# TGAC/KAT

Measured on AMD Instinct MI355X. Metric: k-mers/sec (whole node) for kat comp reads-vs-assembly k=27, higher is better.
Workload: dtype u64

## Files before the change

kat_amd/csrc/kg_partition.hpp:

```cpp
#pragma once
#include "kg_kernels.hpp"
#include "kg_l1_lean.hpp"

#include <cstddef>
#include <type_traits>

namespace kg {

constexpr int PART_BLOCK = 1024;
constexpr int PART_ITEMS = BASES_PER_LANE;
constexpr int TILE_ITEMS = PART_BLOCK * PART_ITEMS;
constexpr int L1_TILE_BYTES = TILE_ITEMS;
constexpr int L1_TILE_STARTS = L1_TILE_BYTES - CHUNK_OVERLAP;
constexpr int L1_LANES_WITH_STARTS = L1_TILE_STARTS / PART_ITEMS;

__device__ __forceinline__ void lds_barrier() { asm volatile("s_waitcnt lgkmcnt(0)\n\ts_barrier" ::: "memory"); }
__device__ __forceinline__ void spill_put(uint64_t* __restrict__ spill, unsigned long long* __restrict__ spill_n, uint64_t cap, uint64_t key) {
    const unsigned long long at = atomicAdd(spill_n, 1ULL);
    if (at < cap) spill[at] = key;
}

struct PartGeom {
    uint32_t R, S;
    uint32_t P1, P2;
// ... 1140 lines not shown
    static_assert(U == 4, "a lane takes one group of the level-2 buffer: four items");
    const uint32_t S = g.S;
    unsigned long long* rk = reinterpret_cast<unsigned long long*>(lds_raw);
    uint32_t* rc = reinterpret_cast<uint32_t*>(lds_raw + (size_t)S * 8);
    const uint32_t tid = threadIdx.x, lane = tid & 63, wave = tid >> 6;
    unsigned long long* wqk = reinterpret_cast<unsigned long long*>(lds_raw + (size_t)S * 12) + (size_t)wave * QCAP;
    uint32_t* wqs = reinterpret_cast<uint32_t*>(lds_raw + (size_t)S * 12 + (size_t)NW * QCAP * 8) + (size_t)wave * QCAP;
    uint32_t new_distinct = 0;
    u32x4 kq[KP], cq[CP];
    __shared__ unsigned long long s_next_chunk;

    const uint32_t r_hi = g.b_hi * g.P2;
    auto run_end = [&](uint32_t r) -> uint64_t {
        if (bend && (r + 1) % g.P2 == 0) return bend[r / g.P2];
        return off2[r + 1];
    };
    auto next_region = [&](uint32_t from) {
        uint32_t r = from;
        while (r < r_hi && (cnt2 ? cnt2[r] == 0 : off2[r] == run_end(r))) r += gridDim.x;
        return r;
    };
    auto prefetch = [&](uint32_t r) {
        const uint64_t base = (uint64_t)r * S;
#pragma unroll
        for (int u = 0; u < KP; ++u) { const uint32_t i = (u * BLOCK + tid) * 2; kq[u] = *reinterpret_cast<const u32x4*>(t.keys + base + (i < S ? i : 0)); }
#pragma unroll
        for (int u = 0; u < CP; ++u) { const uint32_t i = (u * BLOCK + tid) * 4; cq[u] = *reinterpret_cast<const u32x4*>(t.counts + base + (i < S ? i : 0)); }
    };

    uint32_t r = next_region(g.b_lo * g.P2 + blockIdx.x);
    if (r < r_hi) prefetch(r);
    while (r < r_hi) {
        const uint64_t beg = off2[r], end = cnt2 ? beg + cnt2[r] : run_end(r);
        const uint64_t base = (uint64_t)r * S;
        const unsigned long long t_top = now();
#pragma unroll
        for (int u = 0; u < KP; ++u) { const uint32_t i = (u * BLOCK + tid) * 2; if (i < S) *reinterpret_cast<u32x4*>(rk + i) = kq[u]; }
#pragma unroll
        for (int u = 0; u < CP; ++u) { const uint32_t i = (u * BLOCK + tid) * 4; if (i < S) *reinterpret_cast<u32x4*>(rc + i) = cq[u]; }
        const uint32_t rn = next_region(r + gridDim.x);
        const uint32_t rd1 = r >> g.l2, rd2 = r & (g.P2 - 1);

        for (uint64_t sbeg = beg; sbeg < end; sbeg += seg_len) {
            const uint64_t n_run = (end - sbeg < seg_len ? end - sbeg : seg_len);
            if (tid == 0) s_next_chunk = NW;
            lds_barrier();
#pragma unroll 1
            for (int u = 0; u < CP; ++u) {
                const uint32_t i = (u * BLOCK + tid) * 4;
                if (i >= S) break;
                const u32x4 c = *reinterpret_cast<const u32x4*>(rc + i);
                if (!((c.x | c.y | c.z | c.w) & 0x80000000u)) continue;
#pragma unroll 1
                for (uint32_t j = 0; j < 4; ++j)
                    if (rc[i + j] & 0x80000000u) { rc[i + j] -= 0x80000000u; ovf_add(t, rk[i + j], 0x80000000ULL); }
            }
            lds_barrier();
            st[0] += now() - t_top;

            uint32_t q_n = 0;
            auto add1 = [&](uint32_t slot) { (void)__hip_atomic_fetch_add(&rc[slot], 1u, __ATOMIC_RELAXED, __HIP_MEMORY_SCOPE_WORKGROUP); };
            auto drain_pass = [&](bool fin ) {
                const uint32_t take = q_n < 64 ? q_n : 64;
                q_n -= take;
                bool live = lane < take;
                unsigned long long key = EMPTY; uint32_t slot = 0, budget = 0;
                if (live) { key = wqk[q_n + lane]; const uint32_t s = wqs[q_n + lane]; slot = s & 0xFFFF; budget = s >> 16; }
#pragma unroll 1
                for (int rr = 0; rr < AP2_LANE_PROBES; ++rr) {
                    const int busy = __popcll(__ballot(live));
                    if (busy == 0 || (busy < 8 && (fin || rr >= 4))) break;
                    if (live) {
                        unsigned long long c0 = rk[slot];
                        if (c0 == EMPTY) {
                            c0 = atomicCAS(&rk[slot], (unsigned long long)EMPTY, key);
                            if (c0 == EMPTY) { ++new_distinct; c0 = key; }
                        }
                        if (c0 == key) { add1(slot); live = false; }
                        else {
                            slot = slot + 1 == S ? 0 : slot + 1;
                            if (--budget == 0) { spill_put(spill, spill_n, g.spill_cap, key); live = false; }
                        }
                    }
                }
                const bool lng = live && (fin || S - budget >= (uint32_t)(AP2_LANE_PROBES + NR));
                {
                    const bool back = live && !lng;
                    const unsigned long long m = __ballot(back);
                    if (m) {
                        const uint32_t at = q_n + __builtin_amdgcn_mbcnt_hi((uint32_t)(m >> 32), __builtin_amdgcn_mbcnt_lo((uint32_t)m, 0));
                        if (back) { wqk[at] = key; wqs[at] = slot | (budget << 16); }
                        q_n += (uint32_t)__popcll(m);
                    }
                }
                unsigned long long todo = __ballot(lng);
#pragma unroll 1
                while (todo) {
                    const int src = __ffsll((long long)todo) - 1;
                    todo &= todo - 1;
                    const unsigned long long ck = lane_value((uint64_t)key, src);
                    uint32_t cs = lane_value(slot, src);
                    int cb = (int)lane_value(budget, src);
#pragma unroll 1
                    for (;;) {
                        uint32_t idx = cs + lane; if (idx >= S) idx -= S;
                        const unsigned long long c0 = rk[idx];
                        const unsigned long long mk = __ballot(c0 == ck), me = __ballot(c0 == EMPTY);
                        if (!(mk | me)) {
                            cb -= 64; cs = cs + 64 >= S ? cs + 64 - S : cs + 64;
                            if (cb <= 0) { if (lane == 0) spill_put(spill, spill_n, g.spill_cap, ck); break; }
                            continue;
                        }
                        const int first = __ffsll((long long)(mk | me)) - 1;
                        if (first >= cb) { if (lane == 0) spill_put(spill, spill_n, g.spill_cap, ck); break; }
                        unsigned long long got = ck;
                        if (!((mk >> first) & 1)) {
                            unsigned long long old = EMPTY;
                            if ((int)lane == first) old = atomicCAS(&rk[idx], (unsigned long long)EMPTY, ck);
                            old = lane_value((uint64_t)old, first);
                            if (old == EMPTY) { if ((int)lane == first) ++new_distinct; }
                            else got = old;
                        }
                        if (got == ck) { if ((int)lane == first) add1(idx); break; }
                        cb -= first; cs = cs + first >= S ? cs + first - S : cs + first;
                    }
                }
            };

            const uint64_t n_chunks = (n_run + CH - 1) / CH;
            const uint64_t n_grp = (n_run + 3) >> 2, g0 = sbeg >> 2;
            unsigned long long cur[U];
            u32x4 c_lo, n_lo;
            typename HiGroup<HB>::type c_hi{}, n_hi{};
            bool c_in, n_in;
            const L2Run<HB> run(l2_buf, g0);
            { const uint64_t gi = (uint64_t)wave * 64 + lane; c_in = gi < n_grp; run.load(c_in ? (uint32_t)gi : 0u, c_lo, c_hi); }
            auto grab = [&]() -> uint64_t {
                unsigned long long v = 0;
                if (lane == 0) v = atomicAdd(&s_next_chunk, 1ULL);
                return lane_value((uint64_t)v, 0);
            };
            for (uint64_t c = wave; c < n_chunks;) {
                const unsigned long long t_a = now();
                const uint64_t c_next = DYN ? grab() : c + NW;
                {
                    const uint64_t gi = c_next * 64 + lane;
                    n_in = gi < n_grp;
                    run.load(n_in ? (uint32_t)gi : 0u, n_lo, n_hi);
                }
                uint32_t slot[U];
                bool pend[U];
#pragma unroll
                for (int u = 0; u < U; ++u) {
                    const uint64_t rem = ((uint64_t)hi_of_group<HB>(c_hi, u) << 32) | (u == 0 ? c_lo.x : u == 1 ? c_lo.y : u == 2 ? c_lo.z : c_lo.w);
                    pend[u] = c_in && rem != L2Fmt<HB>::NONE;
                    slot[u] = place_offset(rem, g.pl, S);
                    cur[u] = place_key_d(rd1, rd2, rem, g.pl);
                    if (TEST_SPILL && spill_mod && pend[u] && __umulhi((uint32_t)(mix64(cur[u]) >> 32), spill_mod) == 0) { spill_put(spill, spill_n, g.spill_cap, cur[u]); pend[u] = false; }
                }
                const unsigned long long t_b = now();
#pragma unroll
                for (int rr = 0; rr < NR; ++rr) {
                    unsigned long long seen[U];
#pragma unroll
                    for (int u = 0; u < U; ++u) { seen[u] = EMPTY; if (pend[u]) seen[u] = rk[slot[u]]; }
                    bool claim[U];
#pragma unroll
                    for (int u = 0; u < U; ++u) {
                        const bool hit = pend[u] && seen[u] == cur[u];
                        if (hit) add1(slot[u]);
                        pend[u] = pend[u] && !hit;
                        claim[u] = pend[u] && seen[u] == EMPTY;
                        const uint32_t nx = slot[u] + 1 == S ? 0 : slot[u] + 1;
                        slot[u] = (pend[u] && !claim[u]) ? nx : slot[u];
                    }
                    bool any_claim = false;
#pragma unroll
                    for (int u = 0; u < U; ++u) any_claim = any_claim || claim[u];
                    if (INLINE_CLAIM && __any(any_claim)) {
                        unsigned long long got[U];
#pragma unroll
                        for (int u = 0; u < U; ++u) { got[u] = 0; if (claim[u]) got[u] = atomicCAS(&rk[slot[u]], (unsigned long long)EMPTY, cur[u]); }
#pragma unroll
                        for (int u = 0; u < U; ++u) {
                            if (claim[u]) {
                                if (got[u] == EMPTY) ++new_distinct;
                                const bool mine = got[u] == EMPTY || got[u] == cur[u];
                                if (mine) add1(slot[u]);
                                pend[u] = !mine;
                                if (!mine) slot[u] = slot[u] + 1 == S ? 0 : slot[u] + 1;
                            }
                        }
                    }
                }
                if (STAMP) { __builtin_amdgcn_s_waitcnt(0); }
                const unsigned long long t_c = now();
                unsigned long long pm_u[U];
                uint32_t total = 0;
#pragma unroll
                for (int u = 0; u < U; ++u) { pm_u[u] = __ballot(pend[u]); total += (uint32_t)__popcll(pm_u[u]); }
                if (total <= QCAP - 64) {
                    uint32_t at = q_n;
#pragma unroll
                    for (int u = 0; u < U; ++u) {
                        if (pend[u]) {
                            const uint32_t i = at + __builtin_amdgcn_mbcnt_hi((uint32_t)(pm_u[u] >> 32), __builtin_amdgcn_mbcnt_lo((uint32_t)pm_u[u], 0));
                            wqk[i] = cur[u]; wqs[i] = slot[u] | ((S - NR) << 16);
                        }
                        at += (uint32_t)__popcll(pm_u[u]);
                    }
                    q_n += total;
                } else {
                    uint32_t pm = 0;
#pragma unroll
                    for (int u = 0; u < U; ++u) pm |= pend[u] ? 1u << u : 0u;
#pragma unroll 1
                    for (int it = 0; it < U; ++it) {
                        const bool p = pm & 1;
                        const unsigned long long m = __ballot(p);
                        if (m) {
                            while (q_n > QCAP - 64) drain_pass(false);
                            const uint32_t at = q_n + __builtin_amdgcn_mbcnt_hi((uint32_t)(m >> 32), __builtin_amdgcn_mbcnt_lo((uint32_t)m, 0));
                            if (p) { wqk[at] = cur[0]; wqs[at] = slot[0] | ((S - NR) << 16); }
                            q_n += (uint32_t)__popcll(m);
                        }
                        pm >>= 1;
#pragma unroll
                        for (int u = 0; u + 1 < U; ++u) { cur[u] = cur[u + 1]; slot[u] = slot[u + 1]; }
                    }
                }
                const bool last = c_next >= n_chunks;
                while (q_n > (last ? 0u : 64u)) drain_pass(last);
                c_lo = n_lo; c_hi = n_hi; c_in = n_in;
                c = c_next;
                if (STAMP) { const unsigned long long t_d = now(); st[1] += t_b - t_a; st[2] += t_c - t_b; st[3] += t_d - t_c; }
            }
            if (sbeg + seg_len < end) lds_barrier();
        }
        if (rn < r_hi) prefetch(rn);
        const unsigned long long t_w = now();

        lds_barrier();
        const unsigned long long t_x = now();
#pragma unroll
        for (int u = 0; u < KP; ++u) { const uint32_t i = (u * BLOCK + tid) * 2; if (i < S) *reinterpret_cast<u32x4*>(t.keys + base + i) = *reinterpret_cast<const u32x4*>(rk + i); }
#pragma unroll
        for (int u = 0; u < CP; ++u) { const uint32_t i = (u * BLOCK + tid) * 4; if (i < S) *reinterpret_cast<u32x4*>(t.counts + base + i) = *reinterpret_cast<const u32x4*>(rc + i); }
        lds_barrier();
        if (STAMP) { st[4] += t_x - t_w; st[5] += now() - t_x; st[6] += 1; }
        r = rn;
    }
    if (STAMP && tid == 0 && stamps) for (int i = 0; i < 7; ++i) atomicAdd(&stamps[i], st[i]);
    flush_distinct(t, new_distinct);
}

constexpr int APK_LANE_PROBES = 12;
constexpr uint32_t APK_SLOT_SHIFT = 44;

template <int BLOCK, int KP , int HB, bool INLINE_CLAIM = false, bool TEST_SPILL = false,
          bool PF = true ,
          int NR = 3 ,
          bool STAMP = false ,
          int UG = 1 >
__global__ void __launch_bounds__(BLOCK, 4)
k_p3_apply_pk(DevTable t, PartGeom g, const uint64_t* __restrict__ off2, const uint8_t* __restrict__ l2_buf,
              uint64_t* __restrict__ spill, unsigned long long* __restrict__ spill_n, const uint32_t* __restrict__ cnt2, const uint64_t* __restrict__ bend,
              uint32_t qcap , uint64_t seg_len ,
              uint32_t spill_mod,
              uint32_t zero_fill ) {
    extern __shared__ __attribute__((aligned(16))) unsigned char lds_raw[];
    constexpr int NW = BLOCK / 64, U = 4 * UG;
    constexpr uint32_t CH = 64 * U;
    const uint32_t S = g.S, cb = g.cbits;
    const uint64_t cmask = pk_cmask(cb), half = pk_half(cb), rem_mask = (1ULL << APK_SLOT_SHIFT) - 1;
    unsigned long long* rk = reinterpret_cast<unsigned long long*>(lds_raw);
    const uint32_t tid = threadIdx.x, lane = tid & 63, wave = tid >> 6;
    unsigned long long* wq = rk + S + (size_t)wave * qcap;
    uint32_t new_distinct = 0;
    u32x4 kq[KP];
    __shared__ unsigned long long s_next_chunk;

    const uint32_t r_hi = g.b_hi * g.P2;
    auto run_end = [&](uint32_t r) -> uint64_t {
        if (bend && (r + 1) % g.P2 == 0) return bend[r / g.P2];
        return off2[r + 1];
    };
    auto next_region = [&](uint32_t from) {
        uint32_t r = from;
        while (r < r_hi && !zero_fill && (cnt2 ? cnt2[r] == 0 : off2[r] == run_end(r))) r += gridDim.x;
        return r;
    };
    auto prefetch = [&](uint32_t r) {
        if (zero_fill) return;
        const uint64_t base = (uint64_t)r * S;
#pragma unroll
        for (int u = 0; u < KP; ++u) { const uint32_t i = (u * BLOCK + tid) * 2; kq[u] = *reinterpret_cast<const u32x4*>(t.keys + base + (i < S ? i : 0)); }
    };
    auto next_slot = [&](uint32_t s) -> uint32_t { return s + 1 == S ? 0 : s + 1; };
    uint32_t* rk32 = reinterpret_cast<uint32_t*>(rk);
    auto add1 = [&](uint32_t slot) { (void)__hip_atomic_fetch_add(&rk32[2 * slot], 1u, __ATOMIC_RELAXED, __HIP_MEMORY_SCOPE_WORKGROUP); };

    unsigned long long st[7] = {0, 0, 0, 0, 0, 0, 0};
    auto now = [&]() -> unsigned long long { return STAMP ? (unsigned long long)clock64() : 0ULL; };
    uint32_t r = next_region(g.b_lo * g.P2 + blockIdx.x);
    if (PF && r < r_hi) prefetch(r);
    while (r < r_hi) {
        const uint64_t beg = off2[r], end = cnt2 ? beg + cnt2[r] : run_end(r);
        const uint64_t base = (uint64_t)r * S;
        const unsigned long long t_fill = now();
        if (!PF) prefetch(r);
        if (zero_fill) {
#pragma unroll
            for (int u = 0; u < KP; ++u) { const uint32_t i = (u * BLOCK + tid) * 2; if (i < S) *reinterpret_cast<u32x4*>(rk + i) = u32x4{0u, 0u, 0u, 0u}; }
        } else {
#pragma unroll
            for (int u = 0; u < KP; ++u) { const uint32_t i = (u * BLOCK + tid) * 2; if (i < S) *reinterpret_cast<u32x4*>(rk + i) = kq[u]; }
        }
        const uint32_t rn = next_region(r + gridDim.x);
        const uint32_t rd1 = r >> g.l2, rd2 = r & (g.P2 - 1);
        auto spill_rem = [&](uint64_t rem) { spill_put(spill, spill_n, g.spill_cap, place_key_d(rd1, rd2, rem, g.pl)); };

        for (uint64_t sbeg = beg; sbeg < end; sbeg += seg_len) {
            const uint64_t n_run = (end - sbeg < seg_len ? end - sbeg : seg_len);
            if (tid == 0) s_next_chunk = NW;
            lds_barrier();
            const unsigned long long t_walk = now();
            st[0] += t_walk - t_fill;

            uint32_t q_n = 0;
            auto drain_pass = [&](bool fin ) {
                const unsigned long long t_dr = now();
                struct DrainStamp { unsigned long long& acc; unsigned long long t0; bool on; __device__ ~DrainStamp() { if (on) acc += (unsigned long long)clock64() - t0; } } drain_stamp{st[2], t_dr, STAMP};
                const uint32_t take = q_n < 64 ? q_n : 64;
                q_n -= take;
                bool live = lane < take;
                uint64_t rem = 0; uint32_t slot = 0, budget = 0;
                if (live) {
                    const unsigned long long e = wq[q_n + lane];
                    rem = e & rem_mask; slot = (uint32_t)(e >> APK_SLOT_SHIFT);
                    const uint32_t home = place_offset(rem, g.pl, S);
                    budget = S - (slot >= home ? slot - home : slot + S - home);
                }
#pragma unroll 1
                for (int rr = 0; rr < APK_LANE_PROBES; ++rr) {
                    const int busy = __popcll(__ballot(live));
                    if (busy == 0 || (busy < 8 && (fin || rr >= 4))) break;
                    if (live) {
                        unsigned long long w = rk[slot];
                        if (w == 0) {
                            w = atomicCAS(&rk[slot], 0ULL, (unsigned long long)((rem << cb) | 1ULL));
                            if (w == 0) { ++new_distinct; live = false; }
                        }
                        if (live) {
                            if ((w >> cb) == rem) { add1(slot); live = false; }
                            else {
                                slot = next_slot(slot);
                                if (--budget == 0) { spill_rem(rem); live = false; }
                            }
                        }
                    }
                }
                const bool lng = live && (fin || S - budget >= (uint32_t)(APK_LANE_PROBES + NR));
                {
                    const bool back = live && !lng;
                    const unsigned long long m = __ballot(back);
                    if (m) {
                        const uint32_t at = q_n + __builtin_amdgcn_mbcnt_hi((uint32_t)(m >> 32), __builtin_amdgcn_mbcnt_lo((uint32_t)m, 0));
                        if (back) wq[at] = rem | ((unsigned long long)slot << APK_SLOT_SHIFT);
                        q_n += (uint32_t)__popcll(m);
                    }
                }
                unsigned long long todo = __ballot(lng);
#pragma unroll 1
                while (todo) {
                    const int src = __ffsll((long long)todo) - 1;
                    todo &= todo - 1;
                    const unsigned long long ck = lane_value((uint64_t)rem, src);
                    uint32_t cs = lane_value(slot, src);
                    int cbud = (int)lane_value(budget, src);
#pragma unroll 1
                    for (;;) {
                        uint32_t idx = cs + lane; if (idx >= S) idx -= S;
                        const unsigned long long w = rk[idx];
                        const unsigned long long mk = __ballot(w != 0 && (w >> cb) == ck), me = __ballot(w == 0);
                        if (!(mk | me)) {
                            cbud -= 64; cs = cs + 64 >= S ? cs + 64 - S : cs + 64;
                            if (cbud <= 0) { if (lane == 0) spill_rem(ck); break; }
                            continue;
                        }
                        const int first = __ffsll((long long)(mk | me)) - 1;
                        if (first >= cbud) { if (lane == 0) spill_rem(ck); break; }
                        if ((mk >> first) & 1) { if ((int)lane == first) add1(idx); break; }
                        unsigned long long old = 0;
                        if ((int)lane == first) old = atomicCAS(&rk[idx], 0ULL, (unsigned long long)((ck << cb) | 1ULL));
                        old = lane_value((uint64_t)old, first);
                        if (old == 0) { if ((int)lane == first) ++new_distinct; break; }
                        if ((old >> cb) == ck) { if ((int)lane == first) add1(idx); break; }
                        cbud -= first; cs = cs + first >= S ? cs + first - S : cs + first;
                    }
                }
            };

            const uint64_t n_chunks = (n_run + CH - 1) / CH;
            const uint64_t n_grp = (n_run + 3) >> 2, g0 = sbeg >> 2;
            u32x4 c_lo[UG], n_lo[UG];
            typename HiGroup<HB>::type c_hi[UG], n_hi[UG];
            bool c_in[UG], n_in[UG];
            const L2Run<HB> run(l2_buf, g0);
#pragma unroll
            for (int gq = 0; gq < UG; ++gq) {
                const uint64_t gi = ((uint64_t)wave * UG + gq) * 64 + lane;
                c_in[gq] = gi < n_grp; c_hi[gq] = typename HiGroup<HB>::type{}; n_hi[gq] = typename HiGroup<HB>::type{};
                run.load(c_in[gq] ? (uint32_t)gi : 0u, c_lo[gq], c_hi[gq]);
            }
            auto grab = [&]() -> uint64_t {
                unsigned long long v = 0;
                if (lane == 0) v = atomicAdd(&s_next_chunk, 1ULL);
                return lane_value((uint64_t)v, 0);
            };
            for (uint64_t c = wave; c < n_chunks;) {
                const uint64_t c_next = grab();
#pragma unroll
                for (int gq = 0; gq < UG; ++gq) {
                    const uint64_t gi = (c_next * UG + gq) * 64 + lane;
                    n_in[gq] = gi < n_grp;
                    run.load(n_in[gq] ? (uint32_t)gi : 0u, n_lo[gq], n_hi[gq]);
                }
                uint64_t rem[U];
                uint32_t slot[U];
                bool pend[U];
#pragma unroll
                for (int u = 0; u < U; ++u) {
                    const int gq = u >> 2, q = u & 3;
                    rem[u] = ((uint64_t)hi_of_group<HB>(c_hi[gq], q) << 32) | (q == 0 ? c_lo[gq].x : q == 1 ? c_lo[gq].y : q == 2 ? c_lo[gq].z : c_lo[gq].w);
                    pend[u] = c_in[gq] && rem[u] != L2Fmt<HB>::NONE;
                    slot[u] = place_offset(rem[u], g.pl, S);
                    if (TEST_SPILL && spill_mod && pend[u] && __umulhi((uint32_t)(mix64(place_key_d(rd1, rd2, rem[u], g.pl)) >> 32), spill_mod) == 0) { spill_rem(rem[u]); pend[u] = false; }
                }
#pragma unroll
                for (int rr = 0; rr < NR; ++rr) {
                    unsigned long long seen[U];
#pragma unroll
                    for (int u = 0; u < U; ++u) seen[u] = rk[slot[u]];
                    bool claim[U];
#pragma unroll
                    for (int u = 0; u < U; ++u) {
                        const bool hit = pend[u] && seen[u] != 0 && (seen[u] >> cb) == rem[u];
                        (void)__hip_atomic_fetch_add(&rk32[2 * slot[u]], hit ? 1u : 0u, __ATOMIC_RELAXED, __HIP_MEMORY_SCOPE_WORKGROUP);
                        pend[u] = pend[u] && !hit;
                        claim[u] = pend[u] && seen[u] == 0;
                        slot[u] = (pend[u] && !claim[u]) ? next_slot(slot[u]) : slot[u];
                    }
                    bool any_claim = false;
#pragma unroll
                    for (int u = 0; u < U; ++u) any_claim = any_claim || claim[u];
                    if (INLINE_CLAIM && __any(any_claim)) {
                        unsigned long long got[U];
#pragma unroll
                        for (int u = 0; u < U; ++u) { got[u] = 0; if (claim[u]) got[u] = atomicCAS(&rk[slot[u]], 0ULL, (unsigned long long)((rem[u] << cb) | 1ULL)); }
#pragma unroll
                        for (int u = 0; u < U; ++u) {
                            if (claim[u]) {
                                if (got[u] == 0) { ++new_distinct; pend[u] = false; }
                                else if ((got[u] >> cb) == rem[u]) { add1(slot[u]); pend[u] = false; }
                                else slot[u] = next_slot(slot[u]);
                            }
                        }
                    }
                }
                unsigned long long pm_u[U];
                uint32_t total = 0;
#pragma unroll
                for (int u = 0; u < U; ++u) { pm_u[u] = __ballot(pend[u]); total += (uint32_t)__popcll(pm_u[u]); }
                if (UG > 1) while (q_n && q_n + total > qcap) drain_pass(false);
                if (q_n + total <= qcap) {
                    uint32_t at = q_n;
#pragma unroll
                    for (int u = 0; u < U; ++u) {
                        if (pend[u]) wq[at + __builtin_amdgcn_mbcnt_hi((uint32_t)(pm_u[u] >> 32), __builtin_amdgcn_mbcnt_lo((uint32_t)pm_u[u], 0))] = rem[u] | ((unsigned long long)slot[u] << APK_SLOT_SHIFT);
                        at += (uint32_t)__popcll(pm_u[u]);
                    }
                    q_n += total;
                } else {
                    uint32_t pm = 0;
#pragma unroll
                    for (int u = 0; u < U; ++u) pm |= pend[u] ? 1u << u : 0u;
#pragma unroll 1
                    for (int it = 0; it < U; ++it) {
                        const bool p = pm & 1;
                        const unsigned long long m = __ballot(p);
                        if (m) {
                            while (q_n > qcap - 64) drain_pass(false);
                            const uint32_t at = q_n + __builtin_amdgcn_mbcnt_hi((uint32_t)(m >> 32), __builtin_amdgcn_mbcnt_lo((uint32_t)m, 0));
                            if (p) wq[at] = rem[0] | ((unsigned long long)slot[0] << APK_SLOT_SHIFT);
                            q_n += (uint32_t)__popcll(m);
                        }
                        pm >>= 1;
#pragma unroll
                        for (int u = 0; u + 1 < U; ++u) { rem[u] = rem[u + 1]; slot[u] = slot[u + 1]; }
                    }
                }
                const bool last = c_next >= n_chunks;
                while (q_n > (last ? 0u : 64u)) drain_pass(last);
#pragma unroll
                for (int gq = 0; gq < UG; ++gq) { c_lo[gq] = n_lo[gq]; c_hi[gq] = n_hi[gq]; c_in[gq] = n_in[gq]; }
                c = c_next;
                if (STAMP) st[6] += 1;
            }
            const unsigned long long t_post = now();
            st[1] += t_post - t_walk;
            lds_barrier();
            if (sbeg + seg_len < end) {
#pragma unroll 1
                for (int u = 0; u < KP; ++u) {
                    const uint32_t i = (u * BLOCK + tid) * 2;
                    if (i >= S) break;
                    const u64x2 ww = *reinterpret_cast<const u64x2*>(rk + i);
                    if ((ww.x & cmask) <= half && (ww.y & cmask) <= half) continue;
#pragma unroll 1
                    for (uint32_t j = 0; j < 2; ++j) {
                        const unsigned long long w = rk[i + j];
                        const uint64_t c = w & cmask;
                        if (c <= half) continue;
                        const uint64_t keep = ((c - 1) & (half - 1)) + 1;
                        rk[i + j] = w - (c - keep);
                        ovf_add(t, base + i + j, c - keep);
                    }
                }
            }
            if (STAMP) st[3] += now() - t_post;
        }
        if (PF && rn < r_hi) prefetch(rn);

        const unsigned long long t_wb = now();
#pragma unroll
        for (int u = 0; u < KP; ++u) {
            const uint32_t i = (u * BLOCK + tid) * 2;
            if (i < S) {
                u64x2 ww = *reinterpret_cast<const u64x2*>(rk + i);
                if ((ww.x & cmask) > half || (ww.y & cmask) > half) {
                    const uint64_t c0 = ww.x & cmask, c1 = ww.y & cmask;
                    if (c0 > half) { const uint64_t keep = ((c0 - 1) & (half - 1)) + 1; ww.x -= c0 - keep; ovf_add(t, base + i, c0 - keep); }
                    if (c1 > half) { const uint64_t keep = ((c1 - 1) & (half - 1)) + 1; ww.y -= c1 - keep; ovf_add(t, base + i + 1, c1 - keep); }
                }
                *reinterpret_cast<u64x2*>(t.keys + base + i) = ww;
            }
        }
        lds_barrier();
        if (STAMP) { st[4] += now() - t_wb; st[5] += 1; }
        r = rn;
    }
    if (STAMP && tid == 0) { for (int i = 0; i < 7; ++i) atomicAdd(&spill_n[8 + i], st[i]); }
    flush_distinct(t, new_distinct);
}

static __global__ void __launch_bounds__(256)
k_insert_keys(DevTable t, const uint64_t* __restrict__ keys, uint64_t n) {
    uint32_t new_distinct = 0;
    const uint64_t stride = (uint64_t)gridDim.x * blockDim.x;
    for (uint64_t i = (uint64_t)blockIdx.x * blockDim.x + threadIdx.x; i < n; i += stride) {
        if (t.cbits) table_add_pk<true>(t, keys[i], 1ULL, new_distinct);
        else table_add(t, keys[i], 1ULL, new_distinct);
    }
    flush_distinct(t, new_distinct);
}

}
```

Baseline: 100.5 billion.

## Overlap next-region key and first-group loads with writeback of current region

Restructures the per-region loop so that the next region's table-key prefetch and first L2 group loads are issued before the current region's LDS writeback, and the LDS fill for the next region happens after writeback. The overflow split pass now always runs after each segment, which makes the writeback a plain unconditional copy without count checks. The goal is to hide global-load latency behind writeback and trim the writeback loop. The cost is longer live ranges for the c_lo/c_hi registers across iterations, which raises register pressure, plus an extra barrier. The PF template switch is effectively ignored, and out-of-range lanes now write redundantly to index 0.

```diff
diff --git a/kat_amd/csrc/kg_partition.hpp b/kat_amd/csrc/kg_partition.hpp
--- a/kat_amd/csrc/kg_partition.hpp
+++ b/kat_amd/csrc/kg_partition.hpp
@@ -1466,20 +1466,39 @@
 
     unsigned long long st[7] = {0, 0, 0, 0, 0, 0, 0};
     auto now = [&]() -> unsigned long long { return STAMP ? (unsigned long long)clock64() : 0ULL; };
+    auto fill = [&]() {
+        if (zero_fill) {
+#pragma unroll
+            for (int u = 0; u < KP; ++u) { const uint32_t i = (u * BLOCK + tid) * 2; if (i < S) *reinterpret_cast<u32x4*>(rk + i) = u32x4{0u, 0u, 0u, 0u}; }
+        } else {
+#pragma unroll
+            for (int u = 0; u < KP; ++u) { const uint32_t i = (u * BLOCK + tid) * 2; if (i < S) *reinterpret_cast<u32x4*>(rk + i) = kq[u]; }
+        }
+    };
+    u32x4 c_lo[UG];
+    typename HiGroup<HB>::type c_hi[UG];
+    bool c_in[UG];
+    auto first_groups = [&](uint64_t sbeg, uint64_t end) {
+        const uint64_t n_run = (end - sbeg < seg_len ? end - sbeg : seg_len), n_grp = (n_run + 3) >> 2;
+        const L2Run<HB> run(l2_buf, sbeg >> 2);
+#pragma unroll
+        for (int gq = 0; gq < UG; ++gq) {
+            const uint64_t gi = ((uint64_t)wave * UG + gq) * 64 + lane;
+            c_in[gq] = gi < n_grp; c_hi[gq] = typename HiGroup<HB>::type{};
+            run.load(c_in[gq] ? (uint32_t)gi : 0u, c_lo[gq], c_hi[gq]);
+        }
+    };
+    auto region_loads = [&](uint32_t r) {
+        const uint64_t b = off2[r], e = cnt2 ? b + cnt2[r] : run_end(r);
+        if (b < e) first_groups(b, e);
+        prefetch(r);
+    };
     uint32_t r = next_region(g.b_lo * g.P2 + blockIdx.x);
-    if (PF && r < r_hi) prefetch(r);
+    unsigned long long t_fill = now();
+    if (r < r_hi) { region_loads(r); fill(); }
     while (r < r_hi) {
         const uint64_t beg = off2[r], end = cnt2 ? beg + cnt2[r] : run_end(r);
         const uint64_t base = (uint64_t)r * S;
-        const unsigned long long t_fill = now();
-        if (!PF) prefetch(r);
-        if (zero_fill) {
-#pragma unroll
-            for (int u = 0; u < KP; ++u) { const uint32_t i = (u * BLOCK + tid) * 2; if (i < S) *reinterpret_cast<u32x4*>(rk + i) = u32x4{0u, 0u, 0u, 0u}; }
-        } else {
-#pragma unroll
-            for (int u = 0; u < KP; ++u) { const uint32_t i = (u * BLOCK + tid) * 2; if (i < S) *reinterpret_cast<u32x4*>(rk + i) = kq[u]; }
-        }
         const uint32_t rn = next_region(r + gridDim.x);
         const uint32_t rd1 = r >> g.l2, rd2 = r & (g.P2 - 1);
         auto spill_rem = [&](uint64_t rem) { spill_put(spill, spill_n, g.spill_cap, place_key_d(rd1, rd2, rem, g.pl)); };
@@ -1567,16 +1586,13 @@
 
             const uint64_t n_chunks = (n_run + CH - 1) / CH;
             const uint64_t n_grp = (n_run + 3) >> 2, g0 = sbeg >> 2;
-            u32x4 c_lo[UG], n_lo[UG];
-            typename HiGroup<HB>::type c_hi[UG], n_hi[UG];
-            bool c_in[UG], n_in[UG];
+            u32x4 n_lo[UG];
+            typename HiGroup<HB>::type n_hi[UG];
+            bool n_in[UG];
             const L2Run<HB> run(l2_buf, g0);
 #pragma unroll
-            for (int gq = 0; gq < UG; ++gq) {
-                const uint64_t gi = ((uint64_t)wave * UG + gq) * 64 + lane;
-                c_in[gq] = gi < n_grp; c_hi[gq] = typename HiGroup<HB>::type{}; n_hi[gq] = typename HiGroup<HB>::type{};
-                run.load(c_in[gq] ? (uint32_t)gi : 0u, c_lo[gq], c_hi[gq]);
-            }
+            for (int gq = 0; gq < UG; ++gq) n_hi[gq] = typename HiGroup<HB>::type{};
+            if (sbeg != beg) first_groups(sbeg, end);
             auto grab = [&]() -> uint64_t {
                 unsigned long long v = 0;
                 if (lane == 0) v = atomicAdd(&s_next_chunk, 1ULL);
@@ -1674,7 +1690,7 @@
             const unsigned long long t_post = now();
             st[1] += t_post - t_walk;
             lds_barrier();
-            if (sbeg + seg_len < end) {
+            {
 #pragma unroll 1
                 for (int u = 0; u < KP; ++u) {
                     const uint32_t i = (u * BLOCK + tid) * 2;
@@ -1694,24 +1710,18 @@
             }
             if (STAMP) st[3] += now() - t_post;
         }
-        if (PF && rn < r_hi) prefetch(rn);
-
         const unsigned long long t_wb = now();
+        if (rn < r_hi) region_loads(rn);
+        lds_barrier();
 #pragma unroll
         for (int u = 0; u < KP; ++u) {
-            const uint32_t i = (u * BLOCK + tid) * 2;
-            if (i < S) {
-                u64x2 ww = *reinterpret_cast<const u64x2*>(rk + i);
-                if ((ww.x & cmask) > half || (ww.y & cmask) > half) {
-                    const uint64_t c0 = ww.x & cmask, c1 = ww.y & cmask;
-                    if (c0 > half) { const uint64_t keep = ((c0 - 1) & (half - 1)) + 1; ww.x -= c0 - keep; ovf_add(t, base + i, c0 - keep); }
-                    if (c1 > half) { const uint64_t keep = ((c1 - 1) & (half - 1)) + 1; ww.y -= c1 - keep; ovf_add(t, base + i + 1, c1 - keep); }
-                }
-                *reinterpret_cast<u64x2*>(t.keys + base + i) = ww;
-            }
+            const uint32_t i = (u * BLOCK + tid) * 2, ic = i < S ? i : 0u;
+            *reinterpret_cast<u32x4*>(t.keys + base + ic) = *reinterpret_cast<const u32x4*>(rk + ic);
         }
         lds_barrier();
-        if (STAMP) { st[4] += now() - t_wb; st[5] += 1; }
+        t_fill = now();
+        if (STAMP) { st[4] += t_fill - t_wb; st[5] += 1; }
+        if (rn < r_hi) fill();
         r = rn;
     }
     if (STAMP && tid == 0) { for (int i = 0; i < 7; ++i) atomicAdd(&spill_n[8 + i], st[i]); }
```

Result: slower. 98.96 billion (-1.5%).
